# aa217/Neural-Speech-Decoding

Measured on AMD Instinct MI355X. Metric: EEG-trials/sec (train fwd+bwd), higher is better.
Workload: dtype f32; 1 GPU; cfg2: 3-class EEG_LSTM train step (dropout 0.6 + RReLU noise, CE, Adam), 8ch x 250-step windows, H=48 L=2 fp32, batch 256/GPU; batch_per_gpu=256, global_batch=256, T=250, C=8, H=48, L=2, K=3, bidirectional=False, weights=reference checkpoint, parallelism=dp1, launch=eager

## Files before the change

### neural-speech-decoding_amd/csrc/nsd_lstm2_bwd48.hip

```cpp
#include "nsd_args.h"
#include "nsd_multi.h"
#include "nsd_prof.h"
#include "nsd_bf16.h"
#include <type_traits>
#include <utility>

namespace {

constexpr int H = 48;
constexpr int G4 = 192;
constexpr int dl0(const int nb) { return nb == 1 ? 3 : 0; }
constexpr int PRIO1_CHAIN = 2, PRIO1_X1 = 3, PRIO2_CHAIN = 3, PRIO2_X1 = 2, PRIO_LOADER = 1;
constexpr int RING = 8;
constexpr int NTHREADS = 1024;
#ifndef NSD_DW_SLEEP
#define NSD_DW_SLEEP 0
#endif
#ifndef NSD_LD_SLEEP
#define NSD_LD_SLEEP 0
#endif
constexpr int DW_SLEEP = NSD_DW_SLEEP, LD_SLEEP = NSD_LD_SLEEP;
constexpr int CHUNK = 8;
constexpr int REC = 288;
constexpr int REC4 = REC / 4;
constexpr int STAGE_F4 = 2 * CHUNK * REC4;
typedef float f32x4 __attribute__((ext_vector_type(4)));

constexpr int WK = 16;
constexpr int ARS = 224;
constexpr int BRS = 96;
struct DwWin {
    unsigned short wa[2][2][2][WK][ARS];
    unsigned short wb[2][2][2][WK][BRS];
    float pf[2][2][H][8];
    float din1x[8][H];
};
struct NoWin {};
template <int NB>
struct Smem {
    float ring[2][RING][NB][G4];
    float din1[2][NB][H];
    float stage[2][NB][2][CHUNK][REC];
    float xst[2][NB][CHUNK][8];
    typename std::conditional<NB == 1, DwWin, NoWin>::type win;
};

typedef float f32x2 __attribute__((ext_vector_type(2)));
__device__ __forceinline__ f32x2 pk_fma(f32x2 a, f32x2 b, f32x2 c) { return __builtin_elementwise_fma(a, b, c); }

__device__ __forceinline__ float slice_dot_t(const float *dv, const f32x2 (&wp)[4][6]) {
    f32x2 acc[4];
#pragma unroll
    for (int q = 0; q < 3; ++q) {
        const float4 v = *reinterpret_cast<const float4 *>(dv + 4 * q);
        const f32x2 lo = {v.x, v.y}, hi = {v.z, v.w};
#pragma unroll
        for (int jj = 0; jj < 4; ++jj) {
            acc[jj] = q == 0 ? wp[jj][0] * lo : pk_fma(wp[jj][2 * q], lo, acc[jj]);
            acc[jj] = pk_fma(wp[jj][2 * q + 1], hi, acc[jj]);
        }
    }
    const int lane = threadIdx.x;
    const bool odd = (lane & 1) != 0, hi2 = (lane & 2) != 0;
    const float r0 = acc[0].x + acc[0].y, r1 = acc[1].x + acc[1].y;
    const float r2 = acc[2].x + acc[2].y, r3 = acc[3].x + acc[3].y;
    const float ra = (odd ? r1 : r0) + quad_xor1(odd ? r0 : r1);
    const float rb = (odd ? r3 : r2) + quad_xor1(odd ? r2 : r3);
    float v = (hi2 ? rb : ra) + quad_xor2(hi2 ? ra : rb);
    v += row_ror<4>(v);
    v += row_ror<8>(v);
    return v;
}

__device__ __forceinline__ void load_wT(const float *w, const int og, const int kk, f32x2 (&wp)[4][6]) {
#pragma unroll
    for (int jj = 0; jj < 4; ++jj)
#pragma unroll
        for (int p = 0; p < 6; ++p) {
            wp[jj][p].x = w[(size_t)(12 * kk + 2 * p) * H + 4 * og + jj];
            wp[jj][p].y = w[(size_t)(12 * kk + 2 * p + 1) * H + 4 * og + jj];
        }
}

struct PrepIn { float4 gc; float cprev, ct, mk; float2 ad; };
__device__ __forceinline__ PrepIn prep_load(const Lstm2BwdArgs &a, Smem<1> &sm, const int mn, const int layer, const int u, const float cT1) {
    const int T = a.T;
    const int t = layer == 1 ? T - 1 - mn : T + 1 + dl0(1) - mn;
    const float *rec = &sm.stage[(mn >> 3) & 1][0][layer][mn & 7][0];
    const float *recp = &sm.stage[((mn - 1) >> 3) & 1][0][layer][(mn - 1) & 7][0];
    PrepIn in;
    in.gc = *reinterpret_cast<const float4 *>(rec + 4 * u);
    in.cprev = t > 0 ? rec[192 + u] : 0.f;
    in.ct = t == T - 1 ? cT1 : recp[192 + u];
    in.ad = make_float2(0.f, 0.f); in.mk = 1.f;
    if (layer == 1) in.ad = *reinterpret_cast<const float2 *>(rec + 240);
    else if (a.mask || a.rng.on) in.mk = rec[240 + u];
    return in;
}
__device__ __forceinline__ void prep_finish(Smem<1> &sm, const PrepIn &in, const int mn, const int layer, const int u, const float dpu, const float awu) {
    const float ig = in.gc.x, fg = in.gc.y, gg = in.gc.z, og = in.gc.w;
    const float tc = fast_tanh(in.ct);
    const float x = layer == 1 ? fmaf(in.ad.x, dpu, in.ad.y * awu) : in.mk;
    float *o = &sm.win.pf[mn & 1][layer][u][0];
    *reinterpret_cast<float4 *>(o) = make_float4(og * (1.f - tc * tc), fg, x, 0.f);
    *reinterpret_cast<float4 *>(o + 4) = make_float4(gg * (ig * (1.f - ig)), in.cprev * (fg * (1.f - fg)), ig * (1.f - gg * gg), tc * (og * (1.f - og)));
}
__device__ __forceinline__ void prep_layer(const Lstm2BwdArgs &a, Smem<1> &sm, const int mn, const int layer, const int u,
                                           const float dpu, const float awu, const float cT1) {
    const PrepIn in = prep_load(a, sm, mn, layer, u, cT1);
    prep_finish(sm, in, mn, layer, u, dpu, awu);
}

template <int NB, class A>
__device__ __forceinline__ void chain_role(const A &a, Smem<NB> &sm, const int layer, const int r,
                                           const int n_steps) {
    const int og = r >> 4, kk = r & 15;
    const int j = 4 * og + (r & 3), s = (r >> 2) & 3;
    const int T = a.T, B = a.B;
    const float *cseq = layer == 0 ? a.cseq0 : a.cseq1;
    f32x2 wp[4][6];
    load_wT(layer == 0 ? a.w_hh0 : a.w_hh1, og, kk, wp);
    const float awj = a.attn_w[j];
    float db = 0.f;
    Prof prof = prof_init(a.dbg);

    const int ngrp = (B + NB - 1) / NB;
    for (int grp = wg_id(a); grp < ngrp; grp += wg_count(a)) {
        const int b0 = grp * NB;
        float dc[NB], dhrec[NB], ct[NB], dpj[NB];
#pragma unroll
        for (int n = 0; n < NB; ++n) {
            const int b = b0 + n;
            dc[n] = 0.f; dhrec[n] = 0.f;
            dpj[n] = (NB == 2 && layer == 1 && b < B) ? a.dpooled[(size_t)b * H + j] : 0.f;
            ct[n] = (NB == 2 && b < B) ? cseq[((size_t)b * T + (T - 1)) * H + j] : 0.f;
        }
        step_barrier<false>(prof);

        for (int m0 = 0; m0 < n_steps; m0 += CHUNK) {
            const int sb = (m0 / CHUNK) & 1;
#pragma unroll
            for (int k = 0; k < CHUNK; ++k) {
                const int m = m0 + k;
                const int t = layer == 1 ? (T - 1 - m) : (T + 1 + dl0(NB) - m);
                const bool active = (t >= 0 && t < T);
                const bool prev_active = (t + 1 >= 0 && t + 1 < T);
                if constexpr (NB == 1) {
                    const float *pfl = &sm.win.pf[k & 1][layer][j][0];
                    const float4 pf = *reinterpret_cast<const float4 *>(pfl);
                    const float qr = pfl[4 + s];
                    const float dout = layer == 1 ? pf.z : sm.win.din1x[(k + 6 - dl0(NB)) & 7][j] * pf.z;
                    if (prev_active) dhrec[0] = slice_dot_t(&sm.ring[layer][(k + RING - 1) & (RING - 1)][0][12 * kk], wp);
                    if (active) {
                        const float dht = dout + dhrec[0];
                        const float dct = fmaf(dht, pf.x, dc[0]);
                        const float mine = (s == 3 ? dht : dct) * qr;
                        dc[0] = dct * pf.y;
                        db += mine;
                        sm.ring[layer][k][0][s * H + j] = mine;
                    }
                } else
#pragma unroll
                for (int n = 0; n < NB; ++n) {
                    const float *rec = &sm.stage[sb][n][layer][k][0];
                    const float4 gc = *reinterpret_cast<const float4 *>(rec + 4 * j);
                    const float own = rec[4 * j + s];
                    const float cprev = t > 0 ? rec[192 + j] : 0.f;
                    const float aux0 = layer == 1 ? rec[240] : ((a.mask || a.rng.on) ? rec[240 + j] : 1.f);
                    const float aux1 = rec[241];
                    const float ig = gc.x, fg = gc.y, gg = gc.z, og = gc.w;
                    const float tc = fast_tanh(ct[n]);
                    const float wq = og * (1.f - tc * tc);
                    const float dact = s == 2 ? 1.f - own * own : own * (1.f - own);
                    const float qsel = s == 0 ? gg : s == 1 ? cprev : s == 2 ? ig : tc;
                    const float qr = qsel * dact;
                    float dout;
                    if (layer == 1) dout = fmaf(aux0, dpj[n], aux1 * awj);
                    else            dout = sm.din1[(k + 1) & 1][n][j] * aux0;
                    if (prev_active) dhrec[n] = slice_dot_t(&sm.ring[layer][(k + RING - 1) & (RING - 1)][n][12 * kk], wp);
                    if (active) {
                        float mine = 0.f;
                        if (b0 + n < B) {
                            const float dht = dout + dhrec[n];
                            const float dct = fmaf(dht, wq, dc[n]);
                            mine = (s == 3 ? dht : dct) * qr;
                            dc[n] = dct * fg;
                            db += mine;
                            ct[n] = cprev;
                        }
                        sm.ring[layer][k][n][s * H + j] = mine;
                    }
                }
                step_barrier<false>(prof);
            }
        }
    }
    float *slab = a.slabs + (size_t)wg_id(a) * a.slab_stride;
    prof_store(a.dbg, prof);
    if (layer == 0) { slab[a.o_b_ih0 + s * H + j] = db; slab[a.o_b_hh0 + s * H + j] = db; }
    else            { slab[a.o_b_ih1 + s * H + j] = db; slab[a.o_b_hh1 + s * H + j] = db; }
}

template <class A>
__device__ __forceinline__ void x1_role(const A &a, Smem<2> &sm, const int r, const int n_steps) {
    constexpr int NB = 2;
    const int og = r >> 4, kk = r & 15;
    const int j = 4 * og + (r & 3), s = (r >> 2) & 3;
    const int T = a.T, B = a.B, C = a.C;
    f32x2 wp[4][6];
    load_wT(a.w_ih1, og, kk, wp);
    float dWih0[4][2];
#pragma unroll
    for (int g = 0; g < 4; ++g) { dWih0[g][0] = 0.f; dWih0[g][1] = 0.f; }
    const float awj = a.attn_w[j];
    const int c0 = 2 * s, c1 = 2 * s + 1;
    Prof prof = prof_init(a.dbg);

    const int ngrp = (B + NB - 1) / NB;
    for (int grp = wg_id(a); grp < ngrp; grp += wg_count(a)) {
        const int b0 = grp * NB;
        float dpj[NB];
#pragma unroll
        for (int n = 0; n < NB; ++n) dpj[n] = (a.residual && b0 + n < B) ? a.dpooled[(size_t)(b0 + n) * H + j] : 0.f;
        const int pu = (r & 63) < H ? (r & 63) : (r & 63) - 16;
        (void)pu;
        step_barrier<false>(prof);

        for (int m0 = 0; m0 < n_steps; m0 += CHUNK) {
            const int sb = (m0 / CHUNK) & 1;
#pragma unroll
            for (int k = 0; k < CHUNK; ++k) {
                const int m = m0 + k;
                const int t1p = T - m;
                const int t0p = T + 2 - m;
                constexpr int PREV = RING - 1;
                const int e = (k + PREV) & (RING - 1);
#pragma unroll
                for (int n = 0; n < NB; ++n) {
                    const float2 xv = *reinterpret_cast<const float2 *>(&sm.xst[sb][n][k][2 * s]);
                    if (t1p >= 0 && t1p < T) {
                        float inp = slice_dot_t(&sm.ring[1][e][n][12 * kk], wp);
                        if (a.residual && b0 + n < B) {
                            const float *recp = &sm.stage[k == 0 ? sb ^ 1 : sb][n][1][e][0];
                            inp += fmaf(recp[240], dpj[n], recp[241] * awj);
                        }
                        if (s == 0) sm.din1[k & 1][n][j] = inp;
                    }
                    if (t0p >= 0 && t0p < T && b0 + n < B) {
#pragma unroll
                        for (int g = 0; g < 4; ++g) {
                            const float d = sm.ring[0][e][n][g * H + j];
                            dWih0[g][0] = fmaf(d, xv.x, dWih0[g][0]);
                            dWih0[g][1] = fmaf(d, xv.y, dWih0[g][1]);
                        }
                    }
                }
                step_barrier<false>(prof);
            }
        }
    }
    prof_store(a.dbg, prof);
    float *slab = a.slabs + (size_t)wg_id(a) * a.slab_stride;
#pragma unroll
    for (int g = 0; g < 4; ++g) {
        if (c0 < C) slab[a.o_w_ih0 + (size_t)(g * H + j) * C + c0] = dWih0[g][0];
        if (c1 < C) slab[a.o_w_ih0 + (size_t)(g * H + j) * C + c1] = dWih0[g][1];
    }
}

typedef unsigned u32x2v __attribute__((ext_vector_type(2)));
__device__ __forceinline__ float rows_reduce_scatter4(const f32x4 v) {
    const u32x2v p02 = __builtin_amdgcn_permlane32_swap(__float_as_uint(v[0]), __float_as_uint(v[2]), false, false);
    const u32x2v p13 = __builtin_amdgcn_permlane32_swap(__float_as_uint(v[1]), __float_as_uint(v[3]), false, false);
    const float s02 = __uint_as_float(p02[0]) + __uint_as_float(p02[1]);
    const float s13 = __uint_as_float(p13[0]) + __uint_as_float(p13[1]);
    const u32x2v q = __builtin_amdgcn_permlane16_swap(__float_as_uint(s02), __float_as_uint(s13), false, false);
    return __uint_as_float(q[0]) + __uint_as_float(q[1]);
}
template <class A>
__device__ __forceinline__ void x1m_role(const A &a, Smem<1> &sm, const int g, const int lane, const int n_steps) {
    const int T = a.T, B = a.B;
    const int ks = lane >> 4, ub = (lane >> 2) & 3, jc = lane & 3;
    float wv[H];
#pragma unroll
    for (int sidx = 0; sidx < H; ++sidx) wv[sidx] = a.w_ih1[(size_t)(48 * ks + sidx) * H + 16 * g + 4 * ub + jc];
    const int uo = 16 * g + 4 * ub + ks;
    const float awo = a.attn_w[uo];
    const int pu = lane < H ? lane : lane - 16, pl = g == 0 ? 1 : 0;
    const float p_aw = a.attn_w[pu];
    Prof prof = prof_init(a.dbg);
    for (int grp = wg_id(a); grp < B; grp += wg_count(a)) {
        const int b0 = grp;
        const float dpo = a.residual ? a.dpooled[(size_t)b0 * H + uo] : 0.f;
        float p_dp = 0.f, p_c = 0.f;
        if (g < 2) {
            p_dp = a.dpooled[(size_t)b0 * H + pu];
            p_c = (pl == 1 ? a.cseq1 : a.cseq0)[((size_t)b0 * T + (T - 1)) * H + pu];
        }
#pragma unroll
        for (int s4 = 0; s4 < H; s4 += 8)
            asm volatile("" : "+v"(wv[s4]), "+v"(wv[s4 + 1]), "+v"(wv[s4 + 2]), "+v"(wv[s4 + 3]), "+v"(wv[s4 + 4]), "+v"(wv[s4 + 5]), "+v"(wv[s4 + 6]), "+v"(wv[s4 + 7]));
        step_barrier<false>(prof);
        for (int m0 = 0; m0 < n_steps; m0 += CHUNK) {
#pragma unroll
            for (int k = 0; k < CHUNK; ++k) {
                const int m = m0 + k;
                PrepIn pin;
                if (g < 2) pin = prep_load(a, sm, m + 1, pl, pu, p_c);
                if ((k & 3) == 0 && m >= 4) {
                    const float *vj = &sm.ring[1][(k + 4 + jc) & 7][0][48 * ks];
                    f32x4 acc0 = {0.f, 0.f, 0.f, 0.f}, acc1 = acc0, acc2 = acc0, acc3 = acc0;
#pragma unroll
                    for (int qb = 0; qb < 12; qb += 4) {
                        f32x4 bq[4];
#pragma unroll
                        for (int q = 0; q < 4; ++q) bq[q] = *reinterpret_cast<const f32x4 *>(vj + 4 * (qb + q));
#pragma unroll
                        for (int q = 0; q < 4; ++q) {
                            acc0 = __builtin_amdgcn_mfma_f32_4x4x1f32(wv[4 * (qb + q) + 0], bq[q][0], acc0, 0, 0, 0);
                            acc1 = __builtin_amdgcn_mfma_f32_4x4x1f32(wv[4 * (qb + q) + 1], bq[q][1], acc1, 0, 0, 0);
                            acc2 = __builtin_amdgcn_mfma_f32_4x4x1f32(wv[4 * (qb + q) + 2], bq[q][2], acc2, 0, 0, 0);
                            acc3 = __builtin_amdgcn_mfma_f32_4x4x1f32(wv[4 * (qb + q) + 3], bq[q][3], acc3, 0, 0, 0);
                        }
                    }
                    float inp = rows_reduce_scatter4((acc0 + acc1) + (acc2 + acc3));
                    const int c = m - 4 + jc;
                    if (a.residual) {
                        const float *recp = &sm.stage[(c >> 3) & 1][0][1][c & 7][0];
                        inp += fmaf(recp[240], dpo, recp[241] * awo);
                    }
                    sm.win.din1x[(k + 4 + jc) & 7][uo] = inp;
                }
                if (g < 2) prep_finish(sm, pin, m + 1, pl, pu, p_dp, p_aw);
                if (g == 2 && a.da0_out && m >= 1) {
                    const int t0 = T + 2 + dl0(1) - m;
                    if (t0 >= 0 && t0 < T && lane < H)
                        *reinterpret_cast<f32x4 *>(a.da0_out + ((size_t)b0 * T + t0) * G4 + 4 * lane) =
                            *reinterpret_cast<const f32x4 *>(&sm.ring[0][(k + 7) & 7][0][4 * lane]);
                }
                step_barrier<false>(prof);
            }
        }
    }
    prof_store(a.dbg, prof);
}

template <int NB>
// ... 483 lines not shown
```

### neural-speech-decoding_amd/csrc/nsd_lstm2_fwd48.hip

```cpp
#include "nsd_args.h"
#include "nsd_multi.h"
#include "nsd_prof.h"

namespace {

constexpr int H = 48;
constexpr int KS = 12;
constexpr int NT = 768;
constexpr int XCH = 32;
typedef float f32x2 __attribute__((ext_vector_type(2)));
constexpr int SREC = 384;
constexpr int SREC4 = SREC / 4;
constexpr int SRING = 16;
constexpr int SCH = 8;
#ifndef NSD_P_SLEEP
#define NSD_P_SLEEP 2
#endif
#ifndef NSD_S_SLEEP
#define NSD_S_SLEEP 3
#endif
constexpr int P_SLEEP = NSD_P_SLEEP, S_SLEEP = NSD_S_SLEEP;
constexpr int TT_TMAX = 1024, TT_KMAX = 8, TT_W0S = 49;
constexpr int NT_TRAIN = NT;
constexpr int TT_PARTS = NT_TRAIN / 48;

template <int NB>
struct FSmem {
    float xs[2][NB][XCH][8];
    float ms[2][NB][XCH][H];
    float pb[2][NB][4 * H];
    float sv[SRING][NB][2][SREC];
    float pk[NB][8];
    float vec[NB][64];
    float sc[NB][TT_TMAX];
    float w0[64 * TT_W0S];
    float w3[TT_KMAX * 64];
    float vln[64], vx[64], vz[64], vdz[64], vdl[64], dp[64];
    float md[4];
    float red[16];
    float part[TT_PARTS][H];
};

__device__ __forceinline__ f32x2 pk_fma(f32x2 a, f32x2 b, f32x2 c) { return __builtin_elementwise_fma(a, b, c); }

template <int NB>
__device__ __forceinline__ void train_tail(const Lstm2FwdArgs &a, FSmem<NB> &sm, const int tid, const int b, const int n);
template <int NB>
__device__ __forceinline__ void tail_all(const Lstm2FwdArgs &a, FSmem<NB> &sm, const int tid, const int b0);

__device__ __forceinline__ void load_slice(const float *p, f32x2 (&v)[6]) {
#pragma unroll
    for (int q = 0; q < 3; ++q) {
        const float4 u = *reinterpret_cast<const float4 *>(p + 4 * q);
        v[2 * q] = (f32x2){u.x, u.y};
        v[2 * q + 1] = (f32x2){u.z, u.w};
    }
}

__device__ __forceinline__ float reduce_pick(const f32x2 (&acc)[4], const int s) {
    const float r0 = acc[0].x + acc[0].y, r1 = acc[1].x + acc[1].y;
    const float r2 = acc[2].x + acc[2].y, r3 = acc[3].x + acc[3].y;
    const bool odd = (s & 1) != 0, hi = (s & 2) != 0;
    const float ra = (odd ? r1 : r0) + quad_xor1(odd ? r0 : r1);
    const float rb = (odd ? r3 : r2) + quad_xor1(odd ? r2 : r3);
    return (hi ? rb : ra) + quad_xor2(hi ? ra : rb);
}


constexpr float KC = -2.f * LOG2E_F;
constexpr float INV_KC = 1.f / KC;
__host__ __device__ constexpr float gate_scale(const int g) { return g == 2 ? -2.f * LOG2E_F : -LOG2E_F; }

struct CellOut { float gate, c, h; };
__device__ __forceinline__ CellOut cell_step(const float arg, float &cK, const int s, const float hmul) {
    const float r = __builtin_amdgcn_rcpf(1.0f + __builtin_amdgcn_exp2f(arg));
    const float act = s == 2 ? fmaf(2.f * KC, r, -KC) : r;
    const float o = quad_bcast<3>(act);
    const float o2 = (2.f * hmul) * o, on = -hmul * o;
    const float igK = __int_as_float(__builtin_amdgcn_update_dpp(0, __float_as_int(act), QP(0, 0, 0, 0), 0xF, 0xF, true)) * act;
    const float fcK = quad_bcast<1>(act) * cK;
    cK = quad_bcast<2>(igK) + fcK;
    const float rc = __builtin_amdgcn_rcpf(1.0f + __builtin_amdgcn_exp2f(cK));
    CellOut out;
    out.h = fmaf(o2, rc, on);
    out.c = cK * INV_KC;
    out.gate = s == 2 ? act * INV_KC : act;
    return out;
}

template <int NB>
__device__ __forceinline__ float chunk_x_at(const Lstm2FwdArgs &a, const int b0, const int e, const int t0) {
    const int n = e / (XCH * 8), tl = (e >> 3) & (XCH - 1), ch = e & 7;
    const int b = b0 + n, t = t0 + tl;
    return (e < NB * XCH * 8 && b < a.B && t < a.T && ch < a.C) ? a.x[((size_t)b * a.T + t) * a.C + ch] : 0.f;
}
__device__ __forceinline__ float4 chunk_mask_at(const Lstm2FwdArgs &a, const int b0, const int e, const int t0) {
    const int n = e / 384, rem = e - n * 384, tl = rem / 12, q = rem - tl * 12;
    const int b = b0 + n, t = t0 + tl;
    if (a.mask && b < a.B && t < a.T) return *reinterpret_cast<const float4 *>(a.mask + ((size_t)b * a.T + t) * H + 4 * q);
    return make_float4(1.f, 1.f, 1.f, 1.f);
}

template <int NB, class A>
__device__ __forceinline__ void l0_role(const A &a, FSmem<NB> &sm, const int r, const int n_steps) {
    const int j = r >> 2, s = r & 3;
    const int T = a.T, B = a.B, C = a.C;
    f32x2 wx[4], wh[4][6];
#pragma unroll
    for (int g = 0; g < 4; ++g) {
        const int row = g * H + j;
        const float gs = gate_scale(g);
        wx[g].x = (2 * s < C) ? gs * a.w_ih0[(size_t)row * C + 2 * s] : 0.f;
        wx[g].y = (2 * s + 1 < C) ? gs * a.w_ih0[(size_t)row * C + 2 * s + 1] : 0.f;
#pragma unroll
        for (int q = 0; q < 6; ++q) {
            wh[g][q].x = gs * a.w_hh0[(size_t)row * H + s * KS + 2 * q];
            wh[g][q].y = gs * a.w_hh0[(size_t)row * H + s * KS + 2 * q + 1];
        }
    }
    const float biasK = (s == 2 ? gate_scale(2) : gate_scale(0)) * (a.b_ih0[s * H + j] + a.b_hh0[s * H + j]);
    const int hslot = (s == 1) ? 0 : s;
    constexpr int XE = NB * XCH * 8;
    constexpr int XPT = (XE + 191) / 192;
    constexpr int MPT = NB * 2;

    Prof prof = prof_init(a.dbg);
    const int ngrp = (B + NB - 1) / NB;
    for (int grp = wg_id(a); grp < ngrp; grp += wg_count(a)) {
        const int b0 = grp * NB;
        float c[NB];
#pragma unroll
        for (int n = 0; n < NB; ++n) c[n] = 0.f;
        auto x_at = [&](int e, int t0) -> float {
            const int n = e / (XCH * 8), tl = (e >> 3) & (XCH - 1), ch = e & 7;
            const int b = b0 + n, t = t0 + tl;
            return (e < XE && b < B && t < T && ch < C) ? a.x[((size_t)b * T + t) * C + ch] : 0.f;
        };
        auto mask_at = [&](int e, int t0) -> float4 {
            const int n = e / 384, rem = e - n * 384, tl = rem / 12, q = rem - tl * 12;
            const int b = b0 + n, t = t0 + tl;
            if (a.rng.on) {
                float v[4];
#pragma unroll
                for (int u = 0; u < 4; ++u)
                    v[u] = (b < B && t < T && nsd_rand_u32(a.rng.seed, a.rng.base, ((uint64_t)b * T + t) * H + 4 * q + u) < a.rng.thr_lstm)
                               ? 0.f : a.rng.keep_lstm;
                return (b < B && t < T) ? make_float4(v[0], v[1], v[2], v[3]) : make_float4(1.f, 1.f, 1.f, 1.f);
            }
            if (a.mask && b < B && t < T) return *reinterpret_cast<const float4 *>(a.mask + ((size_t)b * T + t) * H + 4 * q);
            return make_float4(1.f, 1.f, 1.f, 1.f);
        };
        for (int e = r; e < SRING * NB * 2 * SREC; e += 192) (&sm.sv[0][0][0][0])[e] = 0.f;
        for (int e = r; e < 2 * NB * 4 * H; e += 192) (&sm.pb[0][0][0])[e] = 0.f;
#pragma unroll
        for (int q = 0; q < XPT; ++q) { const int e = r + 192 * q; if (e < XE) (&sm.xs[0][0][0][0])[e] = x_at(e, 0); }
#pragma unroll
        for (int q = 0; q < MPT; ++q) *reinterpret_cast<float4 *>(&sm.ms[0][0][0][0] + 4 * (r + 192 * q)) = mask_at(r + 192 * q, 0);
        step_barrier<false>(prof);

        for (int m0 = 0; m0 < n_steps; m0 += XCH) {
            const int cb = (m0 / XCH) & 1;
            for (int kh = 0; kh < XCH; kh += SRING) {
#pragma unroll
              for (int kr = 0; kr < SRING; ++kr) {
                const int k = kh + kr;
                const int m = m0 + k;
                if (m < T && !ablated(a.ablate, 64)) {
#pragma unroll
                    for (int n = 0; n < NB; ++n) {
                        const float mk = sm.ms[cb][n][k][j];
                        const float2 xq = *reinterpret_cast<const float2 *>(&sm.xs[cb][n][k][2 * s]);
                        const f32x2 xv = {xq.x, xq.y};
                        f32x2 hv[6];
                        load_slice(&sm.sv[(kr + SRING - 1) & (SRING - 1)][n][0][192 + s * KS], hv);
                        f32x2 acc[4];
#pragma unroll
                        for (int g = 0; g < 4; ++g) {
                            acc[g] = pk_fma(wx[g], xv, (f32x2){g == s ? biasK : 0.f, 0.f});
#pragma unroll
                            for (int q = 0; q < 6; ++q) acc[g] = pk_fma(wh[g][q], hv[q], acc[g]);
                        }
                        const CellOut o = cell_step(reduce_pick(acc, s), c[n], s, s == 2 ? mk : 1.f);
                        float *sr = &sm.sv[kr][n][0][0];
                        sr[192 + 48 * hslot + j] = o.h;
                        sr[192 + 48 + j] = o.c;
                        sr[4 * j + s] = o.gate;
                    }
                }
                step_barrier<false>(prof);
              }
            }
        }
        if (a.head_train) tail_all<NB>(a, sm, threadIdx.x, b0);
        else step_barrier<false>(prof);
    }
    prof_store(a.dbg, prof);
}

template <int NB, class A>
__device__ __forceinline__ void p_role(const A &a, FSmem<NB> &sm, const int r, const int n_steps) {
    const int j = r >> 2, s = r & 3;
    const int T = a.T;
    f32x2 wi[4][6];
#pragma unroll
    for (int g = 0; g < 4; ++g)
#pragma unroll
        for (int q = 0; q < 6; ++q) {
            wi[g][q].x = gate_scale(g) * a.w_ih1[(size_t)(g * H + j) * H + s * KS + 2 * q];
            wi[g][q].y = gate_scale(g) * a.w_ih1[(size_t)(g * H + j) * H + s * KS + 2 * q + 1];
        }
    Prof prof = prof_init(a.dbg);
    const int ngrp = (a.B + NB - 1) / NB;
    for (int grp = wg_id(a); grp < ngrp; grp += wg_count(a)) {
        step_barrier<false>(prof);
        for (int m0 = 0; m0 < n_steps; m0 += SRING) {
#pragma unroll
          for (int k = 0; k < SRING; ++k) {
            const int m = m0 + k;
            if (m >= 1 && m <= T && !ablated(a.ablate, 128)) {
#pragma unroll
                for (int n = 0; n < NB; ++n) {
                    f32x2 iv[6];
                    load_slice(&sm.sv[(k + SRING - 1) & (SRING - 1)][n][0][288 + s * KS], iv);
                    f32x2 acc[4];
#pragma unroll
                    for (int g = 0; g < 4; ++g) {
                        acc[g] = wi[g][0] * iv[0];
#pragma unroll
                        for (int q = 1; q < 6; ++q) acc[g] = pk_fma(wi[g][q], iv[q], acc[g]);
                    }
                    sm.pb[k & 1][n][s * H + j] = reduce_pick(acc, s);
                }
            }
            step_barrier<false, P_SLEEP>(prof);
          }
        }
        if (a.head_train) tail_all<NB>(a, sm, threadIdx.x, grp * NB);
        else step_barrier<false>(prof);
    }
    prof_store(a.dbg, prof);
}

template <int NB, class A>
__device__ __forceinline__ void l1_role(const A &a, FSmem<NB> &sm, const int r, const int n_steps) {
    const int j = r >> 2, s = r & 3;
    const int T = a.T, B = a.B;
    f32x2 wh[4][6];
#pragma unroll
    for (int g = 0; g < 4; ++g)
#pragma unroll
        for (int q = 0; q < 6; ++q) {
            wh[g][q].x = gate_scale(g) * a.w_hh1[(size_t)(g * H + j) * H + s * KS + 2 * q];
            wh[g][q].y = gate_scale(g) * a.w_hh1[(size_t)(g * H + j) * H + s * KS + 2 * q + 1];
        }
    const float biasK = (s == 2 ? gate_scale(2) : gate_scale(0)) * (a.b_ih1[s * H + j] + a.b_hh1[s * H + j]);
    const int hslot = (s == 1) ? 0 : s;
    Prof prof = prof_init(a.dbg);
    const int ngrp = (B + NB - 1) / NB;
    for (int grp = wg_id(a); grp < ngrp; grp += wg_count(a)) {
        float c[NB];
#pragma unroll
        for (int n = 0; n < NB; ++n) c[n] = 0.f;
        step_barrier<false>(prof);
        for (int m0 = 0; m0 < n_steps; m0 += SRING) {
#pragma unroll
          for (int k = 0; k < SRING; ++k) {
            const int m = m0 + k;
            const int t = m - 2;
            prof_mark<-1, false>(prof);
            if (t >= 0 && t < T && !ablated(a.ablate, 1024)) {
                const int prv = (k & 1) ^ 1;
#pragma unroll
                for (int n = 0; n < NB; ++n) {
                    const float pj = sm.pb[prv][n][s * H + j];
                    f32x2 hv[6];
                    load_slice(&sm.sv[(k + SRING - 1) & (SRING - 1)][n][1][192 + s * KS], hv);
                    prof_mark<0, true>(prof);
                    const float pjb = pj + biasK;
                    f32x2 acc[4];
#pragma unroll
                    for (int g = 0; g < 4; ++g) {
                        acc[g] = pk_fma(wh[g][0], hv[0], (f32x2){g == s ? pjb : 0.f, 0.f});
#pragma unroll
                        for (int q = 1; q < 6; ++q) acc[g] = pk_fma(wh[g][q], hv[q], acc[g]);
                    }
                    prof_mark<1, false>(prof);
                    const float arg = reduce_pick(acc, s);
                    prof_mark<2, false>(prof);
                    CellOut o = cell_step(arg, c[n], s, 1.f);
                    prof_mark<4, true>(prof);
                    float *sr = &sm.sv[k][n][1][0];
                    if (a.residual && s == 2) o.h += sm.sv[(k + SRING - 2) & (SRING - 1)][n][0][288 + j];
                    sr[192 + 48 * hslot + j] = o.h;
                    sr[192 + 48 + j] = o.c;
                    sr[4 * j + s] = o.gate;
                    prof_mark<5, false>(prof);
                }
            }
            step_barrier<false>(prof);
          }
        }
        if (a.head_train) tail_all<NB>(a, sm, threadIdx.x, grp * NB);
        else step_barrier<false>(prof);
    }
    prof_store(a.dbg, prof);
}

constexpr int SPIECES = 2 * SCH * SREC4 / 64;

struct SvDesc {
    int dst;
    unsigned meta;
};

template <int NB, class A>
__device__ __forceinline__ void saver_role(const A &a, FSmem<NB> &sm, const int lane, const int n_steps) {
    const int T = a.T;
    SvDesc d[SPIECES];
    float *const sv_base = a.hseq0 ? a.hseq0 : a.top;
#pragma unroll
    for (int q = 0; q < SPIECES; ++q) {
        const int e = q * 64 + lane;
        const int k = e / (2 * SREC4), rem = e - k * (2 * SREC4);
        const int layer = rem / SREC4, w = rem - layer * SREC4;
        const int t0 = k - (layer == 1 ? 2 : 0);
        const int lds_off = (k * NB * 2 + layer) * SREC + 4 * w;
        float *dst = nullptr; int wide = 0;
        if (w < 48)      { dst = layer == 0 ? a.gact0 : a.gact1; wide = 1; if (dst) dst += 4 * w; }
        else if (w < 60) { dst = layer == 0 ? a.hseq0 : a.hseq1; if (dst) dst += 4 * (w - 48); }
        else if (w < 72) { dst = layer == 0 ? a.cseq0 : a.cseq1; if (dst) dst += 4 * (w - 60); }
        else if (w < 84) { dst = layer == 0 ? a.inseq : a.top;   if (dst) dst += 4 * (w - 72); }
        d[q].dst = (dst && sv_base) ? (int)(dst - sv_base) : -1;
        d[q].meta = (unsigned)lds_off | ((unsigned)(t0 + 2) << 16) | ((unsigned)wide << 24);
    }
    Prof prof = prof_init(a.dbg);
    auto flush = [&](const int chunk, const int b0, const int q0, const int q1) {
        const float *ring = &sm.sv[(chunk & 1) * SCH][0][0][0];
#pragma unroll
        for (int qb = 0; qb < SPIECES; qb += 3) {
            if (qb < q0 || qb >= q1) continue;
            float4 v[3][NB];
            bool ok[3];
#pragma unroll
            for (int u = 0; u < 3; ++u) {
                const int q = qb + u;
                const int t = (int)((d[q].meta >> 16) & 0xffu) - 2 + SCH * chunk;
                ok[u] = d[q].dst >= 0 && (unsigned)t < (unsigned)T;
#pragma unroll
                for (int n = 0; n < NB; ++n)
                    v[u][n] = ok[u] ? *reinterpret_cast<const float4 *>(ring + (d[q].meta & 0xffffu) + n * 2 * SREC) : make_float4(0.f, 0.f, 0.f, 0.f);
            }
#pragma unroll
            for (int u = 0; u < 3; ++u) {
                const int q = qb + u;
                const int t = (int)((d[q].meta >> 16) & 0xffu) - 2 + SCH * chunk;
                const unsigned row = (d[q].meta >> 24) & 1u ? 4u * H : (unsigned)H;
#pragma unroll
                for (int n = 0; n < NB; ++n) {
                    const int b = b0 + n;
                    if (ok[u] && b < a.B)
                        *reinterpret_cast<float4 *>(sv_base + d[q].dst + (size_t)((unsigned)(b * T + t)) * row) = v[u][n];
                }
            }
        }
    };
    const int ngrp = (a.B + NB - 1) / NB;
    for (int grp = wg_id(a); grp < ngrp; grp += wg_count(a)) {
        const int b0 = grp * NB;
        step_barrier<false>(prof);
        for (int m0 = 0; m0 < n_steps; m0 += SCH) {
            const int done = m0 / SCH - 1;
            if (done >= 0) flush(done, b0, 0, 3);
            step_barrier<false, S_SLEEP>(prof);
            if (done >= 0) flush(done, b0, 3, 6);
            step_barrier<false, S_SLEEP>(prof);
            if (done >= 0) flush(done, b0, 6, 9);
            step_barrier<false, S_SLEEP>(prof);
            if (done >= 0) flush(done, b0, 9, 12);
            step_barrier<false, S_SLEEP>(prof);
            if (done >= 0) flush(done, b0, 12, 15);
            step_barrier<false, S_SLEEP>(prof);
            if (done >= 0) flush(done, b0, 15, 18);
            step_barrier<false, S_SLEEP>(prof);
            if (done >= 0) flush(done, b0, 18, 21);
            step_barrier<false, S_SLEEP>(prof);
            if (done >= 0) flush(done, b0, 21, 24);
            step_barrier<false, S_SLEEP>(prof);
        }
        flush(n_steps / SCH - 1, b0, 0, SPIECES);
        if (a.head_train) asm volatile("s_waitcnt vmcnt(0)" ::: "memory");
        if (a.head_train) tail_all<NB>(a, sm, threadIdx.x, b0);
        else step_barrier<false>(prof);
    }
    prof_store(a.dbg, prof);
}

struct PoolRun {
    float awp[6], ab;
    float mrun, den, pooled;
    float sc, pkv, scale;
    bool ok, skip;
};
template <int NB>
__device__ __forceinline__ void pool_init(PoolRun &p, const Lstm2FwdArgs &a, const int lane) {
#pragma unroll
    for (int u = 0; u < 6; ++u) p.awp[u] = a.attn_w[6 * (lane & 7) + u];
    p.ab = a.attn_b[0];
}
__device__ __forceinline__ void pool_reset(PoolRun &p) { p.mrun = -INFINITY; p.den = 0.f; p.pooled = 0.f; p.skip = true; }

template <int STAGE, int NB>
__device__ __forceinline__ void pool_stage(PoolRun &p, FSmem<NB> &sm, const int chunk, const int lane, const int T, float *sc_out, const int n = 0) {
    const int kq = lane >> 3, part = lane & 7;
    if (STAGE == 0) {
        const int t = SCH * chunk + kq - 2;
        const float *rec = &sm.sv[(chunk & 1) * SCH + kq][n][1][288];
        float sc = 0.f;
#pragma unroll
        for (int u = 0; u < 6; ++u) sc = fmaf(p.awp[u], rec[6 * part + u], sc);
        sc = oct_sum(sc);
        p.ok = (unsigned)t < (unsigned)T;
        p.sc = p.ok ? sc + p.ab : -INFINITY;
        if (sc_out && p.ok && part == 0) sc_out[t] = p.sc;
    } else if (STAGE == 1) {
        const float cm = rows_combine_max(fmaxf(p.sc, row_ror<8>(p.sc)));
        const float mnew = fmaxf(p.mrun, cm);
        p.skip = (mnew == -INFINITY);
        if (p.skip) return;
        p.pkv = p.ok ? __expf(p.sc - mnew) : 0.f;
        p.scale = __expf(p.mrun - mnew);
        p.mrun = mnew;
    } else if (STAGE == 2) {
        if (p.skip) return;
        const float ps = rows_combine_sum(p.pkv + row_ror<8>(p.pkv));
        p.den = fmaf(p.den, p.scale, ps);
        if (part == 0) sm.pk[n][kq] = p.pkv;
    } else {
        if (p.skip) return;
        float acc = p.pooled * p.scale;
        if (lane < H) {
#pragma unroll
            for (int k = 0; k < SCH; ++k) acc = fmaf(sm.pk[n][k], sm.sv[(chunk & 1) * SCH + k][n][1][288 + lane], acc);
        }
        p.pooled = acc;
    }
}

template <int NB>
__device__ __forceinline__ void pool_loop(PoolRun (&p)[NB], FSmem<NB> &sm, const int lane, const int T, const int n_steps, const bool keep_scores,
                                          Prof &prof) {
    static_assert(NB <= 2, "one pooling stage per step: 4 stages x NB trials per 8-step chunk");
    for (int m0 = 0; m0 < n_steps; m0 += SCH) {
        const int done = m0 / SCH - 1;
#pragma unroll
        for (int n = 0; n < 2; ++n) {
            if (n < NB) {
                float *sc_out = keep_scores ? sm.sc[n < NB ? n : 0] : nullptr;
                if (done >= 0) pool_stage<0, NB>(p[n < NB ? n : 0], sm, done, lane, T, sc_out, n);
                step_barrier<false, S_SLEEP>(prof);
                if (done >= 0) pool_stage<1, NB>(p[n < NB ? n : 0], sm, done, lane, T, sc_out, n);
                step_barrier<false, S_SLEEP>(prof);
                if (done >= 0) pool_stage<2, NB>(p[n < NB ? n : 0], sm, done, lane, T, sc_out, n);
                step_barrier<false, S_SLEEP>(prof);
                if (done >= 0) pool_stage<3, NB>(p[n < NB ? n : 0], sm, done, lane, T, sc_out, n);
                step_barrier<false, S_SLEEP>(prof);
            } else {
#pragma unroll
                for (int k = 0; k < 4; ++k) step_barrier<false, S_SLEEP>(prof);
            }
        }
    }
    const int last = n_steps / SCH - 1;
#pragma unroll
    for (int n = 0; n < NB; ++n) {
        float *sc_out = keep_scores ? sm.sc[n] : nullptr;
        pool_stage<0, NB>(p[n], sm, last, lane, T, sc_out, n);
        pool_stage<1, NB>(p[n], sm, last, lane, T, sc_out, n);
        pool_stage<2, NB>(p[n], sm, last, lane, T, sc_out, n);
        pool_stage<3, NB>(p[n], sm, last, lane, T, sc_out, n);
    }
}

template <int NB, class A>
__device__ __forceinline__ void pool_role(const A &a, FSmem<NB> &sm, const int lane, const int n_steps) {
    static_assert(NB == 1, "inference tail is built for one trial per workgroup");
    const int T = a.T, K = a.K, F = a.F;
    PoolRun pr[NB];
    pool_init<NB>(pr[0], a, lane);
    Prof prof = prof_init(a.dbg);
    const int ngrp = (a.B + NB - 1) / NB;
    for (int grp = wg_id(a); grp < ngrp; grp += wg_count(a)) {
        const int b = grp;
        pool_reset(pr[0]);
        step_barrier<false>(prof);
        pool_loop<NB>(pr, sm, lane, T, n_steps, false, prof);
        const float pooled = pr[0].pooled, den = pr[0].den;
        const float p = lane < H ? pooled / den : 0.f;
        const float mu = wave_sum(p) * (1.0f / H);
        const float dlt = lane < H ? p - mu : 0.f;
        const float rstd = 1.0f / sqrtf(wave_sum(dlt * dlt) * (1.0f / H) + 1e-5f);
        if (lane < H) sm.vec[0][lane] = dlt * rstd * a.ln_w[lane] + a.ln_b[lane];
        float z = 0.f;
        if (lane < F) {
            float acc = a.fc0_b[lane];
            const float *w = a.fc0_w + (size_t)lane * H;
#pragma unroll 8
            for (int j = 0; j < H; ++j) acc = fmaf(w[j], sm.vec[0][j], acc);
            z = acc >= 0.f ? acc : acc * a.eval_slope;
        }
        if (lane < F) sm.vec[0][lane] = z;
        float lg = -INFINITY;
        if (lane < K) {
            float acc = a.fc3_b[lane];
            const float *w = a.fc3_w + (size_t)lane * F;
            for (int f = 0; f < F; ++f) acc = fmaf(w[f], sm.vec[0][f], acc);
            lg = acc;
            if (b < a.B) a.logits_out[(size_t)b * K + lane] = acc;
        }
        if (a.probs_out) {
            const float mx = wave_max(lg);
            const float e = lane < K ? __expf(lg - mx) : 0.f;
            const float d = wave_sum(e);
            if (lane < K && b < a.B) a.probs_out[(size_t)b * K + lane] = e / d;
        }
        step_barrier<false>(prof);
    }
    prof_store(a.dbg, prof);
}


__device__ __forceinline__ float tail_block_sum(float v, float *red, const int tid) {
    v = wave_sum(v);
    if ((tid & 63) == 0) red[tid >> 6] = v;
    __syncthreads();
    float s = 0.f;
#pragma unroll
    for (int w = 0; w < NT_TRAIN / 64; ++w) s += red[w];
    __syncthreads();
    return s;
}

template <int NB>
// ... 332 lines not shown
```

Measured before the change: 1.037 million trials/s.

## Split recurrent step loops into branch-free interior and rolled edge blocks

Adds a ring_block helper that, for NB==1, runs a fully unrolled path with compile-time-true activity predicates when a whole chunk lies inside the valid time window, and a rolled (unroll 1) loop for edge chunks. This is applied to the forward layer-0, projection and layer-1 loops, the backward recurrence loop, and the saver role, whose flush descriptors are restructured to per-step 3-entry tables. A LEAN variant of cell_step uses select-based constants, plus a scheduling barrier, to cut divergent branching. The intent is to remove per-step bounds checks and shrink code or register pressure. The cost is more code paths and possible instruction-cache or register effects.

```diff
diff --git a/neural-speech-decoding_amd/csrc/nsd_lstm2_bwd48.hip b/neural-speech-decoding_amd/csrc/nsd_lstm2_bwd48.hip
--- a/neural-speech-decoding_amd/csrc/nsd_lstm2_bwd48.hip
+++ b/neural-speech-decoding_amd/csrc/nsd_lstm2_bwd48.hip
@@ -1,6 +1,7 @@
 #include "nsd_args.h"
 #include "nsd_multi.h"
 #include "nsd_prof.h"
+#include "nsd_ring_block.h"
 #include "nsd_bf16.h"
 #include <type_traits>
 #include <utility>
@@ -137,14 +138,13 @@
         }
         step_barrier<false>(prof);
 
+        const int tb = layer == 1 ? T - 1 : T + 1 + dl0(NB);
         for (int m0 = 0; m0 < n_steps; m0 += CHUNK) {
             const int sb = (m0 / CHUNK) & 1;
-#pragma unroll
-            for (int k = 0; k < CHUNK; ++k) {
-                const int m = m0 + k;
-                const int t = layer == 1 ? (T - 1 - m) : (T + 1 + dl0(NB) - m);
-                const bool active = (t >= 0 && t < T);
-                const bool prev_active = (t + 1 >= 0 && t + 1 < T);
+            ring_block<NB, CHUNK>(m0 >= tb - T + 2 && m0 + CHUNK - 1 <= tb, [&](const int k, const auto inside) {
+                const int t = tb - (m0 + k);
+                const bool active = inside.value || (t >= 0 && t < T);
+                const bool prev_active = inside.value || (t + 1 >= 0 && t + 1 < T);
                 if constexpr (NB == 1) {
                     const float *pfl = &sm.win.pf[k & 1][layer][j][0];
                     const float4 pf = *reinterpret_cast<const float4 *>(pfl);
@@ -192,7 +192,7 @@
                     }
                 }
                 step_barrier<false>(prof);
-            }
+            });
         }
     }
     float *slab = a.slabs + (size_t)wg_id(a) * a.slab_stride;
diff --git a/neural-speech-decoding_amd/csrc/nsd_lstm2_fwd48.hip b/neural-speech-decoding_amd/csrc/nsd_lstm2_fwd48.hip
--- a/neural-speech-decoding_amd/csrc/nsd_lstm2_fwd48.hip
+++ b/neural-speech-decoding_amd/csrc/nsd_lstm2_fwd48.hip
@@ -1,6 +1,7 @@
 #include "nsd_args.h"
 #include "nsd_multi.h"
 #include "nsd_prof.h"
+#include "nsd_ring_block.h"
 
 namespace {
 
@@ -22,6 +23,11 @@
 constexpr int P_SLEEP = NSD_P_SLEEP, S_SLEEP = NSD_S_SLEEP;
 constexpr int TT_TMAX = 1024, TT_KMAX = 8, TT_W0S = 49;
 constexpr int NT_TRAIN = NT;
+#if NSD_MULTI_TU
+template <int NB> constexpr bool LEAN = false;
+#else
+template <int NB> constexpr bool LEAN = NB == 1;
+#endif
 constexpr int TT_PARTS = NT_TRAIN / 48;
 
 template <int NB>
@@ -72,9 +78,11 @@
 __host__ __device__ constexpr float gate_scale(const int g) { return g == 2 ? -2.f * LOG2E_F : -LOG2E_F; }
 
 struct CellOut { float gate, c, h; };
+template <bool LANEK>
 __device__ __forceinline__ CellOut cell_step(const float arg, float &cK, const int s, const float hmul) {
     const float r = __builtin_amdgcn_rcpf(1.0f + __builtin_amdgcn_exp2f(arg));
-    const float act = s == 2 ? fmaf(2.f * KC, r, -KC) : r;
+    const float act = LANEK ? fmaf(s == 2 ? 2.f * KC : 1.f, r, s == 2 ? -KC : 0.f)
+                            : (s == 2 ? fmaf(2.f * KC, r, -KC) : r);
     const float o = quad_bcast<3>(act);
     const float o2 = (2.f * hmul) * o, on = -hmul * o;
     const float igK = __int_as_float(__builtin_amdgcn_update_dpp(0, __float_as_int(act), QP(0, 0, 0, 0), 0xF, 0xF, true)) * act;
@@ -84,7 +92,7 @@
     CellOut out;
     out.h = fmaf(o2, rc, on);
     out.c = cK * INV_KC;
-    out.gate = s == 2 ? act * INV_KC : act;
+    out.gate = LANEK ? act * (s == 2 ? INV_KC : 1.f) : (s == 2 ? act * INV_KC : act);
     return out;
 }
 
@@ -158,37 +166,37 @@
         for (int q = 0; q < MPT; ++q) *reinterpret_cast<float4 *>(&sm.ms[0][0][0][0] + 4 * (r + 192 * q)) = mask_at(r + 192 * q, 0);
         step_barrier<false>(prof);
 
+        auto step = [&](const int cb, const int k, const int kr) {
+#pragma unroll
+            for (int n = 0; n < NB; ++n) {
+                float mk = sm.ms[cb][n][k][j];
+                const float2 xq = *reinterpret_cast<const float2 *>(&sm.xs[cb][n][k][2 * s]);
+                const f32x2 xv = {xq.x, xq.y};
+                f32x2 hv[6];
+                load_slice(&sm.sv[(kr + SRING - 1) & (SRING - 1)][n][0][192 + s * KS], hv);
+                if constexpr (LEAN<NB>) { asm volatile("" : "+v"(mk)); __builtin_amdgcn_sched_barrier(0); }
+                f32x2 acc[4];
+#pragma unroll
+                for (int g = 0; g < 4; ++g) {
+                    acc[g] = pk_fma(wx[g], xv, (f32x2){g == s ? biasK : 0.f, 0.f});
+#pragma unroll
+                    for (int q = 0; q < 6; ++q) acc[g] = pk_fma(wh[g][q], hv[q], acc[g]);
+                }
+                const CellOut o = cell_step<LEAN<NB>>(reduce_pick(acc, s), c[n], s, s == 2 ? mk : 1.f);
+                float *sr = &sm.sv[kr][n][0][0];
+                sr[192 + 48 * hslot + j] = o.h;
+                sr[192 + 48 + j] = o.c;
+                sr[4 * j + s] = o.gate;
+            }
+        };
         for (int m0 = 0; m0 < n_steps; m0 += XCH) {
             const int cb = (m0 / XCH) & 1;
             for (int kh = 0; kh < XCH; kh += SRING) {
-#pragma unroll
-              for (int kr = 0; kr < SRING; ++kr) {
-                const int k = kh + kr;
-                const int m = m0 + k;
-                if (m < T && !ablated(a.ablate, 64)) {
-#pragma unroll
-                    for (int n = 0; n < NB; ++n) {
-                        const float mk = sm.ms[cb][n][k][j];
-                        const float2 xq = *reinterpret_cast<const float2 *>(&sm.xs[cb][n][k][2 * s]);
-                        const f32x2 xv = {xq.x, xq.y};
-                        f32x2 hv[6];
-                        load_slice(&sm.sv[(kr + SRING - 1) & (SRING - 1)][n][0][192 + s * KS], hv);
-                        f32x2 acc[4];
-#pragma unroll
-                        for (int g = 0; g < 4; ++g) {
-                            acc[g] = pk_fma(wx[g], xv, (f32x2){g == s ? biasK : 0.f, 0.f});
-#pragma unroll
-                            for (int q = 0; q < 6; ++q) acc[g] = pk_fma(wh[g][q], hv[q], acc[g]);
-                        }
-                        const CellOut o = cell_step(reduce_pick(acc, s), c[n], s, s == 2 ? mk : 1.f);
-                        float *sr = &sm.sv[kr][n][0][0];
-                        sr[192 + 48 * hslot + j] = o.h;
-                        sr[192 + 48 + j] = o.c;
-                        sr[4 * j + s] = o.gate;
-                    }
-                }
-                step_barrier<false>(prof);
-              }
+              const int mb = m0 + kh;
+              ring_block<NB, SRING>(mb + SRING <= T, [&](const int kr, const auto inside) {
+                  if ((inside.value || mb + kr < T) && !ablated(a.ablate, 64)) step(cb, kh + kr, kr);
+                  step_barrier<false>(prof);
+              });
             }
         }
         if (a.head_train) tail_all<NB>(a, sm, threadIdx.x, b0);
@@ -213,27 +221,26 @@
     const int ngrp = (a.B + NB - 1) / NB;
     for (int grp = wg_id(a); grp < ngrp; grp += wg_count(a)) {
         step_barrier<false>(prof);
+        auto step = [&](const int k) {
+#pragma unroll
+            for (int n = 0; n < NB; ++n) {
+                f32x2 iv[6];
+                load_slice(&sm.sv[(k + SRING - 1) & (SRING - 1)][n][0][288 + s * KS], iv);
+                f32x2 acc[4];
+#pragma unroll
+                for (int g = 0; g < 4; ++g) {
+                    acc[g] = wi[g][0] * iv[0];
+#pragma unroll
+                    for (int q = 1; q < 6; ++q) acc[g] = pk_fma(wi[g][q], iv[q], acc[g]);
+                }
+                sm.pb[k & 1][n][s * H + j] = reduce_pick(acc, s);
+            }
+        };
         for (int m0 = 0; m0 < n_steps; m0 += SRING) {
-#pragma unroll
-          for (int k = 0; k < SRING; ++k) {
-            const int m = m0 + k;
-            if (m >= 1 && m <= T && !ablated(a.ablate, 128)) {
-#pragma unroll
-                for (int n = 0; n < NB; ++n) {
-                    f32x2 iv[6];
-                    load_slice(&sm.sv[(k + SRING - 1) & (SRING - 1)][n][0][288 + s * KS], iv);
-                    f32x2 acc[4];
-#pragma unroll
-                    for (int g = 0; g < 4; ++g) {
-                        acc[g] = wi[g][0] * iv[0];
-#pragma unroll
-                        for (int q = 1; q < 6; ++q) acc[g] = pk_fma(wi[g][q], iv[q], acc[g]);
-                    }
-                    sm.pb[k & 1][n][s * H + j] = reduce_pick(acc, s);
-                }
-            }
-            step_barrier<false, P_SLEEP>(prof);
-          }
+          ring_block<NB, SRING>(m0 >= 1 && m0 + SRING <= T + 1, [&](const int k, const auto inside) {
+              if ((inside.value || (m0 + k >= 1 && m0 + k <= T)) && !ablated(a.ablate, 128)) step(k);
+              step_barrier<false, P_SLEEP>(prof);
+          });
         }
         if (a.head_train) tail_all<NB>(a, sm, threadIdx.x, grp * NB);
         else step_barrier<false>(prof);
@@ -262,43 +269,43 @@
 #pragma unroll
         for (int n = 0; n < NB; ++n) c[n] = 0.f;
         step_barrier<false>(prof);
+        const bool res = a.residual != 0;
+        auto step = [&](const int k) {
+            const int prv = (k & 1) ^ 1;
+#pragma unroll
+            for (int n = 0; n < NB; ++n) {
+                const float pj = sm.pb[prv][n][s * H + j];
+                f32x2 hv[6];
+                load_slice(&sm.sv[(k + SRING - 1) & (SRING - 1)][n][1][192 + s * KS], hv);
+                prof_mark<0, true>(prof);
+                const float pjb = pj + biasK;
+                f32x2 acc[4];
+#pragma unroll
+                for (int g = 0; g < 4; ++g) {
+                    acc[g] = pk_fma(wh[g][0], hv[0], (f32x2){g == s ? pjb : 0.f, 0.f});
+#pragma unroll
+                    for (int q = 1; q < 6; ++q) acc[g] = pk_fma(wh[g][q], hv[q], acc[g]);
+                }
+                prof_mark<1, false>(prof);
+                const float arg = reduce_pick(acc, s);
+                prof_mark<2, false>(prof);
+                CellOut o = cell_step<LEAN<NB>>(arg, c[n], s, 1.f);
+                prof_mark<4, true>(prof);
+                float *sr = &sm.sv[k][n][1][0];
+                if (res && s == 2) o.h += sm.sv[(k + SRING - 2) & (SRING - 1)][n][0][288 + j];
+                sr[192 + 48 * hslot + j] = o.h;
+                sr[192 + 48 + j] = o.c;
+                sr[4 * j + s] = o.gate;
+                prof_mark<5, false>(prof);
+            }
+        };
         for (int m0 = 0; m0 < n_steps; m0 += SRING) {
-#pragma unroll
-          for (int k = 0; k < SRING; ++k) {
-            const int m = m0 + k;
-            const int t = m - 2;
-            prof_mark<-1, false>(prof);
-            if (t >= 0 && t < T && !ablated(a.ablate, 1024)) {
-                const int prv = (k & 1) ^ 1;
-#pragma unroll
-                for (int n = 0; n < NB; ++n) {
-                    const float pj = sm.pb[prv][n][s * H + j];
-                    f32x2 hv[6];
-                    load_slice(&sm.sv[(k + SRING - 1) & (SRING - 1)][n][1][192 + s * KS], hv);
-                    prof_mark<0, true>(prof);
-                    const float pjb = pj + biasK;
-                    f32x2 acc[4];
-#pragma unroll
-                    for (int g = 0; g < 4; ++g) {
-                        acc[g] = pk_fma(wh[g][0], hv[0], (f32x2){g == s ? pjb : 0.f, 0.f});
-#pragma unroll
-                        for (int q = 1; q < 6; ++q) acc[g] = pk_fma(wh[g][q], hv[q], acc[g]);
-                    }
-                    prof_mark<1, false>(prof);
-                    const float arg = reduce_pick(acc, s);
-                    prof_mark<2, false>(prof);
-                    CellOut o = cell_step(arg, c[n], s, 1.f);
-                    prof_mark<4, true>(prof);
-                    float *sr = &sm.sv[k][n][1][0];
-                    if (a.residual && s == 2) o.h += sm.sv[(k + SRING - 2) & (SRING - 1)][n][0][288 + j];
-                    sr[192 + 48 * hslot + j] = o.h;
-                    sr[192 + 48 + j] = o.c;
-                    sr[4 * j + s] = o.gate;
-                    prof_mark<5, false>(prof);
-                }
-            }
-            step_barrier<false>(prof);
-          }
+          const bool in_window = m0 >= 2 && m0 + SRING <= T + 2;
+          ring_block<NB, SRING>(in_window, [&](const int k, const auto inside) {
+              prof_mark<-1, false>(prof);
+              if ((inside.value || (m0 + k >= 2 && m0 + k < T + 2)) && !ablated(a.ablate, 1024)) step(k);
+              step_barrier<false>(prof);
+          });
         }
         if (a.head_train) tail_all<NB>(a, sm, threadIdx.x, grp * NB);
         else step_barrier<false>(prof);
@@ -306,61 +313,52 @@
     prof_store(a.dbg, prof);
 }
 
-constexpr int SPIECES = 2 * SCH * SREC4 / 64;
-
 struct SvDesc {
-    int dst;
-    unsigned meta;
+    float *dst;
+    int ring;
+    unsigned row;
+    int lag;
 };
 
 template <int NB, class A>
 __device__ __forceinline__ void saver_role(const A &a, FSmem<NB> &sm, const int lane, const int n_steps) {
     const int T = a.T;
-    SvDesc d[SPIECES];
-    float *const sv_base = a.hseq0 ? a.hseq0 : a.top;
-#pragma unroll
-    for (int q = 0; q < SPIECES; ++q) {
-        const int e = q * 64 + lane;
-        const int k = e / (2 * SREC4), rem = e - k * (2 * SREC4);
+    SvDesc d[3];
+#pragma unroll
+    for (int u = 0; u < 3; ++u) {
+        const int rem = u * 64 + lane;
         const int layer = rem / SREC4, w = rem - layer * SREC4;
-        const int t0 = k - (layer == 1 ? 2 : 0);
-        const int lds_off = (k * NB * 2 + layer) * SREC + 4 * w;
-        float *dst = nullptr; int wide = 0;
-        if (w < 48)      { dst = layer == 0 ? a.gact0 : a.gact1; wide = 1; if (dst) dst += 4 * w; }
+        float *dst = nullptr; unsigned row = H;
+        if (w < 48)      { dst = layer == 0 ? a.gact0 : a.gact1; row = 4 * H; if (dst) dst += 4 * w; }
         else if (w < 60) { dst = layer == 0 ? a.hseq0 : a.hseq1; if (dst) dst += 4 * (w - 48); }
         else if (w < 72) { dst = layer == 0 ? a.cseq0 : a.cseq1; if (dst) dst += 4 * (w - 60); }
         else if (w < 84) { dst = layer == 0 ? a.inseq : a.top;   if (dst) dst += 4 * (w - 72); }
-        d[q].dst = (dst && sv_base) ? (int)(dst - sv_base) : -1;
-        d[q].meta = (unsigned)lds_off | ((unsigned)(t0 + 2) << 16) | ((unsigned)wide << 24);
+        d[u].lag = 2 * layer;
+        d[u].row = (dst && (a.hseq0 || a.top)) ? row : 0u;
+        d[u].ring = layer * SREC + 4 * w;
+        d[u].dst = dst ? dst - (size_t)d[u].lag * row : nullptr;
     }
     Prof prof = prof_init(a.dbg);
-    auto flush = [&](const int chunk, const int b0, const int q0, const int q1) {
-        const float *ring = &sm.sv[(chunk & 1) * SCH][0][0][0];
-#pragma unroll
-        for (int qb = 0; qb < SPIECES; qb += 3) {
-            if (qb < q0 || qb >= q1) continue;
-            float4 v[3][NB];
-            bool ok[3];
-#pragma unroll
-            for (int u = 0; u < 3; ++u) {
-                const int q = qb + u;
-                const int t = (int)((d[q].meta >> 16) & 0xffu) - 2 + SCH * chunk;
-                ok[u] = d[q].dst >= 0 && (unsigned)t < (unsigned)T;
-#pragma unroll
-                for (int n = 0; n < NB; ++n)
-                    v[u][n] = ok[u] ? *reinterpret_cast<const float4 *>(ring + (d[q].meta & 0xffffu) + n * 2 * SREC) : make_float4(0.f, 0.f, 0.f, 0.f);
-            }
-#pragma unroll
-            for (int u = 0; u < 3; ++u) {
-                const int q = qb + u;
-                const int t = (int)((d[q].meta >> 16) & 0xffu) - 2 + SCH * chunk;
-                const unsigned row = (d[q].meta >> 24) & 1u ? 4u * H : (unsigned)H;
-#pragma unroll
-                for (int n = 0; n < NB; ++n) {
-                    const int b = b0 + n;
-                    if (ok[u] && b < a.B)
-                        *reinterpret_cast<float4 *>(sv_base + d[q].dst + (size_t)((unsigned)(b * T + t)) * row) = v[u][n];
-                }
+    auto flush = [&](auto edge, const int chunk, const int b0, const int k) {
+        constexpr bool EDGE = decltype(edge)::value;
+        const float *ring = &sm.sv[(chunk & 1) * SCH][0][0][0] + k * (NB * 2 * SREC);
+        const int mk = SCH * chunk + k;
+        float4 v[3][NB];
+        bool ok[3];
+#pragma unroll
+        for (int u = 0; u < 3; ++u) {
+            ok[u] = d[u].row != 0u && (!EDGE || (unsigned)(mk - d[u].lag) < (unsigned)T);
+#pragma unroll
+            for (int n = 0; n < NB; ++n)
+                v[u][n] = ok[u] ? *reinterpret_cast<const float4 *>(ring + d[u].ring + n * 2 * SREC) : make_float4(0.f, 0.f, 0.f, 0.f);
+        }
+#pragma unroll
+        for (int u = 0; u < 3; ++u) {
+#pragma unroll
+            for (int n = 0; n < NB; ++n) {
+                const int b = b0 + n;
+                if (ok[u] && b < a.B)
+                    *reinterpret_cast<float4 *>(d[u].dst + (size_t)((unsigned)(b * T + mk)) * d[u].row) = v[u][n];
             }
         }
     };
@@ -370,24 +368,22 @@
         step_barrier<false>(prof);
         for (int m0 = 0; m0 < n_steps; m0 += SCH) {
             const int done = m0 / SCH - 1;
-            if (done >= 0) flush(done, b0, 0, 3);
-            step_barrier<false, S_SLEEP>(prof);
-            if (done >= 0) flush(done, b0, 3, 6);
-            step_barrier<false, S_SLEEP>(prof);
-            if (done >= 0) flush(done, b0, 6, 9);
-            step_barrier<false, S_SLEEP>(prof);
-            if (done >= 0) flush(done, b0, 9, 12);
-            step_barrier<false, S_SLEEP>(prof);
-            if (done >= 0) flush(done, b0, 12, 15);
-            step_barrier<false, S_SLEEP>(prof);
-            if (done >= 0) flush(done, b0, 15, 18);
-            step_barrier<false, S_SLEEP>(prof);
-            if (done >= 0) flush(done, b0, 18, 21);
-            step_barrier<false, S_SLEEP>(prof);
-            if (done >= 0) flush(done, b0, 21, 24);
-            step_barrier<false, S_SLEEP>(prof);
-        }
-        flush(n_steps / SCH - 1, b0, 0, SPIECES);
+            if (done >= 1 && SCH * done + SCH <= T) {
+#pragma unroll
+                for (int k = 0; k < SCH; ++k) {
+                    flush(std::false_type{}, done, b0, k);
+                    step_barrier<false, S_SLEEP>(prof);
+                }
+            } else {
+#pragma unroll 1
+                for (int k = 0; k < SCH; ++k) {
+                    if (done >= 0) flush(std::true_type{}, done, b0, k);
+                    step_barrier<false, S_SLEEP>(prof);
+                }
+            }
+        }
+#pragma unroll 1
+        for (int k = 0; k < SCH; ++k) flush(std::true_type{}, n_steps / SCH - 1, b0, k);
         if (a.head_train) asm volatile("s_waitcnt vmcnt(0)" ::: "memory");
         if (a.head_train) tail_all<NB>(a, sm, threadIdx.x, b0);
         else step_barrier<false>(prof);
diff --git a/neural-speech-decoding_amd/csrc/nsd_ring_block.h b/neural-speech-decoding_amd/csrc/nsd_ring_block.h
--- /dev/null
+++ b/neural-speech-decoding_amd/csrc/nsd_ring_block.h
@@ -0,0 +1,19 @@
+#pragma once
+#include <hip/hip_runtime.h>
+#include <type_traits>
+
+template <int NB, int N, class Body>
+__device__ __forceinline__ void ring_block(const bool inside, Body &&body) {
+    if constexpr (NB == 1) {
+        if (inside) {
+#pragma unroll
+            for (int k = 0; k < N; ++k) body(k, std::true_type{});
+        } else {
+#pragma unroll 1
+            for (int k = 0; k < N; ++k) body(k, std::false_type{});
+        }
+    } else {
+#pragma unroll
+        for (int k = 0; k < N; ++k) body(k, std::false_type{});
+    }
+}
```

After: 1.100 million trials/s (median of 6 runs). 1.06x the previous value.
